# KolinGuo/MPlib

Hardware: AMD Instinct MI355X
Metric: configs/sec full collide() Panda-7DoF+10 boxes (higher is better)
Workload: dtype f64; 1 GPU; cfg3 panda_10boxes: 1048576 configs/GPU/step, 129 pairs, full self+world collide() with ACM filter; configs_per_gpu=1048576, pairs=129, mask_words=5, parallelism=dp1 (config shards, no data-path collective)

## Files before the change

include/mpgpu.h:

```cpp
#ifndef MPGPU_H
#define MPGPU_H

#include <stddef.h>
#include <stdint.h>

#ifdef __cplusplus
extern "C" {
#endif

#define MPG_VERSION_MAJOR 0
#define MPG_VERSION_MINOR 3

#define MPG_OK 0
#define MPG_E_INVALID 1
#define MPG_E_UNSUPPORTED 2
#define MPG_E_HIP 3
#define MPG_E_NOMEM 4
#define MPG_E_FAILED 5

#define MPG_MEM_HOST 0
#define MPG_MEM_DEVICE 1

#define MPG_JOINT_RX 0
#define MPG_JOINT_RY 1
// ... 206 lines not shown
#define MPG_SCREW_TRUNCATED 16
#define MPG_SCREW_SINGULAR 32
#define MPG_SCREW_ROT_PI 64

typedef struct mpg_screw_options {
  double qpos_step;
  int32_t max_waypoints;
} mpg_screw_options;

int mpg_screw_batch(mpg_world *world, int32_t link, const double *goal ,
                    const double *q_start , int64_t rows,
                    const mpg_screw_options *opt , double *path ,
                    int32_t *n_waypoints , uint8_t *status ,
                    int32_t *first_hit , int mem, void *stream);

int mpg_fcl_bvh_build(const double *vertices, int32_t n_vertices, const int32_t *triangles, int32_t n_triangles,
                      double *boxes, int32_t *links, int32_t *leaf_order);

int mpg_debug_sincos(const double *x, int64_t n, double *s, double *c, int device);

int mpg_latency_server_stats(mpg_world *world, int64_t *served, int64_t *starts, int64_t *fallbacks,
                             int32_t *state);

int mpg_synchronize(int device);

int mpg_device_count(int *count);
const char *mpg_last_error(void);
int mpg_last_error_copy(char *buf, size_t size);
const char *mpg_version(void);

#ifdef __cplusplus
}
#endif
#endif
```

mplib_amd/_capi.py:

```python
from __future__ import annotations

import ctypes
import os

_HERE = os.path.dirname(os.path.abspath(__file__))
LIB_PATH = os.path.join(_HERE, "lib", "libmpgpu.so")

MPG_OK, MPG_E_INVALID, MPG_E_UNSUPPORTED, MPG_E_HIP, MPG_E_NOMEM, MPG_E_FAILED = 0, 1, 2, 3, 4, 5
MPG_MEM_HOST, MPG_MEM_DEVICE = 0, 1
STAGES = ("cull", "bucket", "narrow")

(JOINT_RX, JOINT_RY, JOINT_RZ, JOINT_REVOLUTE_UNALIGNED, JOINT_PX, JOINT_PY, JOINT_PZ,
 JOINT_PRISMATIC_UNALIGNED, JOINT_RUBX, JOINT_RUBY, JOINT_RUBZ, JOINT_RUB_UNALIGNED) = range(12)
GEOM_CONVEX, GEOM_BOX, GEOM_SPHERE, GEOM_CAPSULE, GEOM_CYLINDER, GEOM_OCTREE, GEOM_MESH, GEOM_ELLIPSOID, GEOM_CONE = range(9)
GJK_LIBCCD, GJK_INDEP = 0, 1
LINK_FREE = -1

_I32P = ctypes.POINTER(ctypes.c_int32)
_F64P = ctypes.POINTER(ctypes.c_double)
_U8P = ctypes.POINTER(ctypes.c_uint8)
_U32P = ctypes.POINTER(ctypes.c_uint32)


class WorldDesc(ctypes.Structure):
# ... 117 lines not shown
                                                 ctypes.c_int64, ctypes.c_int, ctypes.c_void_p, ctypes.c_void_p,
                                                 ctypes.c_void_p, ctypes.c_void_p, ctypes.c_void_p, ctypes.c_int,
                                                 ctypes.c_void_p]),
    "mpg_fk_batch": (ctypes.c_int, [ctypes.c_void_p, ctypes.c_void_p, ctypes.c_int64, ctypes.c_void_p,
                                    ctypes.c_int, ctypes.c_void_p]),
    "mpg_ik_batch": (ctypes.c_int, [ctypes.c_void_p, ctypes.c_int32, ctypes.c_void_p, ctypes.c_int64, ctypes.c_int64,
                                    ctypes.c_void_p, ctypes.c_void_p, ctypes.POINTER(IkOptions), ctypes.c_void_p,
                                    ctypes.c_void_p, ctypes.c_void_p, ctypes.c_void_p, ctypes.c_int, ctypes.c_void_p]),
    "mpg_screw_batch": (ctypes.c_int, [ctypes.c_void_p, ctypes.c_int32, ctypes.c_void_p, ctypes.c_void_p, ctypes.c_int64,
                                       ctypes.POINTER(ScrewOptions), ctypes.c_void_p, ctypes.c_void_p, ctypes.c_void_p,
                                       ctypes.c_void_p, ctypes.c_int, ctypes.c_void_p]),
    "mpg_profile_enable": (ctypes.c_int, [ctypes.c_void_p, ctypes.c_int]),
    "mpg_profile_read": (ctypes.c_int, [ctypes.c_void_p, ctypes.POINTER(ctypes.c_double),
                                        ctypes.POINTER(ctypes.c_int64), ctypes.POINTER(ctypes.c_int64), ctypes.c_int]),
    "mpg_debug_collide_pairs": (ctypes.c_int, [ctypes.c_void_p, ctypes.c_int32, ctypes.c_int32, ctypes.c_int64,
                                                ctypes.c_void_p, ctypes.c_void_p, ctypes.c_void_p]),
    "mpg_debug_sincos": (ctypes.c_int, [ctypes.c_void_p, ctypes.c_int64, ctypes.c_void_p, ctypes.c_void_p,
                                        ctypes.c_int]),
    "mpg_fcl_bvh_build": (ctypes.c_int, [ctypes.c_void_p, ctypes.c_int32, ctypes.c_void_p, ctypes.c_int32,
                                         ctypes.c_void_p, ctypes.c_void_p, ctypes.c_void_p]),
    "mpg_latency_server_stats": (ctypes.c_int, [ctypes.c_void_p, ctypes.POINTER(ctypes.c_int64),
                                                ctypes.POINTER(ctypes.c_int64), ctypes.POINTER(ctypes.c_int64),
                                                ctypes.POINTER(ctypes.c_int32)]),
    "mpg_synchronize": (ctypes.c_int, [ctypes.c_int]),
    "mpg_device_count": (ctypes.c_int, [ctypes.POINTER(ctypes.c_int)]),
    "mpg_last_error": (ctypes.c_char_p, []),
    "mpg_last_error_copy": (ctypes.c_int, [ctypes.c_char_p, ctypes.c_size_t]),
    "mpg_version": (ctypes.c_char_p, []),
}

_lib = None


class MpgError(RuntimeError):
    pass


def lib() -> ctypes.CDLL:
    global _lib
    if _lib is None:
        if not os.path.exists(LIB_PATH):
            raise ImportError(f"mplib_amd: HIP library {LIB_PATH} is missing -- run `make -C mplib_amd` "
                              "(there is no CPU fallback)")
        try:
            import torch
        except ImportError:
# ... 19 lines not shown
```

mplib_amd/batch.py:

```python
from __future__ import annotations

import ctypes
from typing import Dict, Optional

import numpy as np

from . import _capi as C

_DESC_INT_FIELDS = ["joint_type", "joint_parent", "joint_q_source", "link_parent", "geom_type",
                    "geom_vertex_start", "geom_vertex_count", "moving_link", "moving_geom", "static_geom",
                    "pair_a", "pair_b"]
_DESC_F64_FIELDS = ["joint_axis", "joint_placement", "joint_q_const", "link_placement", "geom_param",
                    "vertices", "moving_offset", "static_transform"]


class DeviceWorld:

    def __init__(self, arrays: Dict[str, np.ndarray], device: int = 0, gjk_tolerance: float = 1e-6,
                 gjk_solver: int = C.GJK_LIBCCD):
        L = C.lib()
        self._keep = []

        def ip(name):
            a = np.ascontiguousarray(np.asarray(arrays[name], dtype=np.int32).reshape(-1))
# ... 67 lines not shown
        nf, far = ctypes.c_int32(0), ctypes.c_double(0.0)
        C.check(L.mpg_world_get_free_info(h, ctypes.byref(nf), ctypes.byref(far), None), "mpg_world_get_free_info")
        self.n_free = nf.value
        self.far_radius = far.value

    def close(self):
        if getattr(self, "_h", None):
            C.lib().mpg_world_destroy(self._h)
            self._h = None

    def __del__(self):
        try:
            self.close()
        except Exception:
            pass

    @property
    def handle(self):
        return self._h

    def set_small_batch_max(self, n: int):
        C.check(C.lib().mpg_set_small_batch_max(self._h, int(n)), "mpg_set_small_batch_max")

    def release_stream(self, stream: int):
        C.check(C.lib().mpg_release_stream(self._h, ctypes.c_void_p(int(stream))), "mpg_release_stream")

    def collide_batch(self, q, flags=None, pair_mask=None, stream: Optional[int] = None, free_pose=None):
        if hasattr(q, "data_ptr"):
            n = q.shape[0] if q.dim() > 1 else q.numel() // self.dof
            if flags is None:
                raise ValueError("device path needs preallocated flags (and optionally pair_mask)")
            mk = ctypes.c_void_p(pair_mask.data_ptr() if pair_mask is not None else 0)
            if free_pose is not None:
                rows = self._free_rows(free_pose.numel(), n)
                C.check(C.lib().mpg_collide_batch_free(self._h, ctypes.c_void_p(q.data_ptr()),
                                                       ctypes.c_void_p(free_pose.data_ptr()), rows, n,
                                                       ctypes.c_void_p(flags.data_ptr()), mk, C.MPG_MEM_DEVICE,
                                                       ctypes.c_void_p(stream or 0)), "mpg_collide_batch_free")
                return flags, pair_mask
            C.check(C.lib().mpg_collide_batch(self._h, ctypes.c_void_p(q.data_ptr()), n,
                                              ctypes.c_void_p(flags.data_ptr()), mk,
                                              C.MPG_MEM_DEVICE, ctypes.c_void_p(stream or 0)), "mpg_collide_batch")
            return flags, pair_mask
        qa = np.ascontiguousarray(np.asarray(q, dtype=np.float64)).reshape(-1, self.dof)
        n = qa.shape[0]
        fl = np.zeros(n, np.uint8)
# ... 183 lines not shown
```

mplib_amd/csrc/mpg_abi_world.h:

```cpp
#pragma once

const char* mpg_last_error(void) { return g_last_error.c_str(); }

int mpg_fcl_bvh_build(const double* vertices, int32_t n_vertices, const int32_t* triangles, int32_t n_triangles,
                      double* boxes, int32_t* links, int32_t* leaf_order) {
  if (n_triangles <= 0 || !vertices || !triangles || !boxes || !links || !leaf_order)
    return set_error(MPG_E_INVALID, "mpg_fcl_bvh_build: empty mesh or NULL buffer");
  for (int64_t i = 0; i < 3 * (int64_t)n_triangles; ++i)
    if (triangles[i] < 0 || triangles[i] >= n_vertices) return set_error(MPG_E_INVALID, "triangle vertex out of range");
  FclBvh B;
  B.box.resize(FB_STRIDE);
  B.link.resize(3);
  std::vector<int> prim((size_t)n_triangles);
  for (int t = 0; t < n_triangles; ++t) prim[t] = t;
  fcl_bvh_node(B, vertices, triangles, prim, 0, 0, n_triangles, 0);
  std::copy(B.box.begin(), B.box.end(), boxes);
  std::copy(B.link.begin(), B.link.end(), links);
  std::copy(prim.begin(), prim.end(), leaf_order);
  return (int)(B.link.size() / 3);
}

int mpg_last_error_copy(char* buf, size_t size) {
  const size_t len = g_last_error.size();
  if (buf && size > 0) {
// ... 46 lines not shown
  for (auto& mk : w->marks) {
    w->ev_pool.push_back(std::move(mk.a));
    w->ev_pool.push_back(std::move(mk.b));
  }
  w->marks.clear();
  for (int k = 0; k < MPG_NUM_STAGES; ++k) {
    if (k < n_stages) {
      if (ms) ms[k] = w->prof_ms[k];
      if (launches) launches[k] = w->prof_n[k];
      if (units) units[k] = u[k];
    }
    w->prof_ms[k] = 0.0;
    w->prof_n[k] = 0;
  }
  return MPG_OK;
}

int mpg_latency_server_stats(mpg_world* w, int64_t* served, int64_t* starts, int64_t* fallbacks, int32_t* state) {
  if (!w) return set_error(MPG_E_INVALID, "world is NULL");
  if (served) *served = w->srv_served;
  if (starts) *starts = w->srv_starts;
  if (fallbacks) *fallbacks = w->srv_fallbacks;
  if (state) *state = !(w->srv_mode && w->srv_ok) ? 0 : w->srv_broken ? 2 : 1;
  return MPG_OK;
}

int mpg_synchronize(int device) {
  HIP_TRY(hipSetDevice(device));
  HIP_TRY(hipDeviceSynchronize());
  return MPG_OK;
}

int mpg_world_create(const mpg_world_desc* d_in, int device, mpg_world** out) {
  if (!out) return set_error(MPG_E_INVALID, "out is NULL");
  *out = nullptr;
  int rc = validate(d_in);
  if (rc) return rc;
  mpg_world_desc dd = *d_in;
  std::vector<int32_t> lp_kin(dd.link_parent, dd.link_parent + dd.n_links);
  int n_free = 0;
  for (int32_t& p : lp_kin)
    if (p == MPG_LINK_FREE) {
      p = 0;
      ++n_free;
    }
  if (n_free) dd.link_parent = lp_kin.data();
// ... 312 lines not shown
  for (int m = 0; m < d->n_moving; ++m) off = std::max(off, std::sqrt(sq3(d->moving_offset + 12 * m + 9)));
  for (int g = 0; g < d->n_geoms; ++g) geo_r = std::max(geo_r, geom_rec[G_STRIDE * g + G_RADIUS] +
                                                                   std::sqrt(sq3(&geom_rec[G_STRIDE * g + G_OBB_C])));
  for (int s2 = 0; s2 < d->n_static; ++s2) stat_x = std::max(stat_x, std::sqrt(sq3(d->static_transform + 12 * s2 + 9)));
  double X = std::max(reach_x + off, stat_x) + geo_r;
  bp_margin = std::max(bp_margin, (float)(kFp32CullRel * X));
  double small_margin = may_mpr ? std::max(kSmallMargin, reach) : kSmallMargin;
  double far_r = 0.0;
  if (n_free) {
    const double link_r = std::sqrt(3.0) * reach_x + off + geo_r;
    const float quat_slack = (float)(4.0 * kFreeQuatTol * geo_r);
    bp_margin += quat_slack;
    small_margin += 4.0 * kFreeQuatTol * geo_r;
    for (int it = 0; it < 8; ++it) {
      far_r = (link_r + (double)bp_margin + 1e-6 * (1.0 + X)) * (1.0 + 1e-9);
      X = std::max(X, far_r + 2.0 * geo_r);
      bp_margin = std::max(bp_margin, (float)(kFp32CullRel * X) + quat_slack);
    }
    far_r = (link_r + (double)bp_margin + 1e-6 * (1.0 + X)) * (1.0 + 1e-9);
    X = std::max(X, far_r + 2.0 * geo_r);
  }
  const double pose_bound = reach_x;
  std::vector<std::array<double, 4>> ball(std::max(d->n_moving, 1));
  for (int m = 0; m < d->n_moving; ++m) {
    const int l = d->moving_link[m];
    const double* g = geom_rec.data() + G_STRIDE * d->moving_geom[m];
    const double* mo = d->moving_offset + 12 * m;
    const double* lp = d->link_placement + 12 * l;
    double a[3], bpt[3];
    for (int i = 0; i < 3; ++i)
      a[i] = mo[3 * i] * g[G_OBB_C] + mo[3 * i + 1] * g[G_OBB_C + 1] + mo[3 * i + 2] * g[G_OBB_C + 2] + mo[9 + i];
    for (int i = 0; i < 3; ++i) bpt[i] = lp[3 * i] * a[0] + lp[3 * i + 1] * a[1] + lp[3 * i + 2] * a[2] + lp[9 + i];
    const int cs = chain_start[l], cn = chain_len[l];
    double R = g[G_RADIUS];
    if (cn == 0) {
      ball[m] = {bpt[0], bpt[1], bpt[2], R};
      continue;
    }
    const int j1 = chain_joints[cs] - 1;
    const double* p1 = d->joint_placement + 12 * j1 + 9;
    R += travel[j1] + std::sqrt(sq3(bpt));
    for (int k = 1; k < cn; ++k) {
      const int j = chain_joints[cs + k] - 1;
      R += std::sqrt(sq3(d->joint_placement + 12 * j + 9)) + travel[j];
    }
    ball[m] = {p1[0], p1[1], p1[2], R * (1.0 + 1e-9) + 1e-9};
  }
  auto never_near = [&](int m, int sid) {
    const double* sr = static_rec.data() + (size_t)S_STRIDE * sid;
    const double* gs = geom_rec.data() + G_STRIDE * d->static_geom[sid];
    double e2 = 0.0;
    for (int k = 0; k < 3; ++k) {
      double t = 0.0;
      for (int i = 0; i < 3; ++i) t += (ball[m][i] - sr[S_OBBC + i]) * sr[S_R + 3 * i + k];
      const double ex = std::max(std::fabs(t) - gs[G_OBB_E + k], 0.0);
      e2 += ex * ex;
    }
    const double slack = 1e-6 * (1.0 + X);
    return std::sqrt(e2) - ball[m][3] > (double)bp_margin + slack;
  };
  std::vector<int> all_mask(std::max(W, 1), 0);
  for (int p = 0; p < d->n_pairs; ++p)
    if (!allowed[p]) all_mask[p >> 5] |= (int)(1u << (p & 31));
  const int ns = d->n_static;
  std::vector<int> sched_start(d->n_moving + 1, 0), sched_pair, sched_other, st_start(2 * (ns + 1), 0), st_m;
  std::vector<float> st_r;
  for (int m = 0; m < d->n_moving; ++m) {
    sched_start[m] = (int)sched_pair.size();
    for (int p = 0; p < d->n_pairs; ++p) {
// ... 4 lines not shown
      sched_pair.push_back(p);
      sched_other.push_back(hi);
      st_m.push_back(0);
      st_r.push_back(0.f);
    }
  }
  sched_start[d->n_moving] = (int)sched_pair.size();
  for (int g = 0; g < 2; ++g) {
    for (int sid = 0; sid < ns; ++sid) {
      st_start[g * (ns + 1) + sid] = (int)sched_pair.size();
      for (int m = 0; m < d->n_moving; ++m)
        for (int p = 0; p < d->n_pairs; ++p) {
          if (allowed[p]) continue;
          const int a = d->pair_a[p], b = d->pair_b[p];
          if (std::min(a, b) != m || std::max(a, b) != d->n_moving + sid) continue;
          if (never_near(m, sid) != (g == 1)) continue;
          sched_pair.push_back(p);
          sched_other.push_back(d->n_moving + sid);
          st_m.push_back(m);
          st_r.push_back(bpp.mobj[BM_STRIDE * m + BM_R]);
        }
    }
    st_start[g * (ns + 1) + ns] = (int)sched_pair.size();
  }
  if (sched_pair.empty()) {
    sched_pair.push_back(0);
    sched_other.push_back(0);
    st_m.push_back(0);
    st_r.push_back(0.f);
  }

  BlobBuilder bb;
  const size_t o_jt = bb.add(d->joint_type, d->n_joints);
  const size_t o_jp = bb.add(d->joint_parent, d->n_joints);
  const size_t o_jqs = bb.add(d->joint_q_source, d->n_joints);
  const size_t o_jqc = bb.add(d->joint_q_const, d->n_joints);
  const size_t o_ja = bb.add(d->joint_axis, 3 * (size_t)d->n_joints);
  const size_t o_jpl = bb.add(d->joint_placement, 12 * (size_t)d->n_joints);
  const size_t o_lp = bb.add(d->link_parent, d->n_links);
  const size_t o_lpl = bb.add(d->link_placement, 12 * (size_t)d->n_links);
  const size_t o_gt = bb.add(d->geom_type, d->n_geoms);
  const size_t o_gvs = bb.add(gstart.data(), gstart.size());
  const size_t o_gnv = bb.add(ngroups.data(), ngroups.size());
  std::vector<int> nvert(std::max(d->n_geoms, 1), 0);
  for (int g = 0; g < d->n_geoms; ++g) nvert[g] = d->geom_type[g] == MPG_GEOM_CONVEX ? d->geom_vertex_count[g] : 0;
  const size_t o_gnvt = bb.add(nvert.data(), nvert.size());
// ... 62 lines not shown
    r[SR_SH] = (bpp.pair_sh[2 * p] + 2) | ((bpp.pair_sh[2 * p + 1] + 2) << 16);
  }
  const size_t o_srr = bb.add(sched_rec.data(), sched_rec.size());
  const size_t o_olf = bb.add(oct_leaf.data(), oct_leaf.size());
  const size_t o_mtr = bb.add(mesh_tri.data(), mesh_tri.size());
  const size_t o_mnd = bb.add(mesh_node.data(), mesh_node.size());
  const size_t o_mln = bb.add(mesh_link.data(), mesh_link.size());
  const size_t o_mtt = bb.add(mesh_tree.data(), mesh_tree.size());
  const size_t o_lrec = bb.add(lat_rec.data(), lat_rec.size());
  const size_t o_fbb = bb.add(fbvh.box.data(), fbvh.box.size());
  const size_t o_fbl = bb.add(fbvh.link.data(), fbvh.link.size());
  const size_t o_fbr = bb.add(fb_root.data(), fb_root.size());
  const size_t o_tps = bb.add(tri_pos.data(), tri_pos.size());
  const size_t o_sob = bb.add(sobb.data(), sobb.size());
  const size_t o_ogr = bb.add(oct_grid.data(), oct_grid.size());
  const size_t o_oce = bb.add(oct_cells.data(), oct_cells.size());
  const size_t o_oli = bb.add(oct_list.data(), oct_list.size());
  const size_t o_opa = bb.add(oct_path.data(), oct_path.size());
  const size_t o_ode = bb.add(oct_depth.data(), oct_depth.size());
  std::vector<int> free_obj(n_free, 0);
  for (int m = 0; m < d->n_moving; ++m)
    if (d->moving_link[m] >= d->n_links - n_free) free_obj[d->moving_link[m] - (d->n_links - n_free)] = m;
  const size_t o_fob = n_free ? bb.add(free_obj.data(), free_obj.size()) : 0;

  std::unique_ptr<mpg_world> w(new mpg_world());
  w->device = device;
  w->n_geoms = d->n_geoms;
  w->geom_type_h.assign(d->geom_type, d->geom_type + d->n_geoms);
  w->block = block;
  w->lds_bytes = lds;
  w->blob_bytes = bb.bytes.size();
  {
    uint64_t h = 1469598103934665603ull;
    for (const char c : bb.bytes) h = (h ^ (uint8_t)c) * 1099511628211ull;
    w->snapshot_hash = h;
  }
  HIP_TRY(w->blob.reserve(w->blob_bytes));
  HIP_TRY(hipMemcpy(w->blob.get(), bb.bytes.data(), w->blob_bytes, hipMemcpyHostToDevice));
  char* base = w->blob.get();
  DevWorld& dw = w->dw;
  dw.nj = d->n_joints;
  dw.dof = d->dof;
  dw.n_links = d->n_links;
  dw.n_geoms = d->n_geoms;
  dw.n_moving = d->n_moving;
  dw.n_static = d->n_static;
// ... 96 lines not shown
    w->has_closed_form |= pair_cf[p] != CF_NONE && !allowed[p];
    w->has_octree |= pair_cf[p] == CF_OCTREE && !allowed[p];
    w->octree_first |= pair_cf[p] == CF_OCTREE && !allowed[p] && obj_geom_type(d, d->pair_a[p]) == MPG_GEOM_OCTREE;
    w->any_closed_form |= pair_cf[p] != CF_NONE && cf_class(pair_cf[p]) == CLS_CLOSED;
    w->any_octree |= pair_cf[p] == CF_OCTREE;
    w->has_mesh |= pair_cf[p] == CF_MESH && !allowed[p];
    w->any_mesh |= pair_cf[p] == CF_MESH;
    w->any_gjk |= pair_cf[p] == CF_GJK;
    w->has_octree2 |= !allowed[p] && obj_geom_type(d, d->pair_a[p]) == MPG_GEOM_OCTREE &&
                      obj_geom_type(d, d->pair_b[p]) == MPG_GEOM_OCTREE;
  }
  dw.static_T = to_cptr<double>(base + o_sT);
  dw.link_chain_start = to_cptr<int>(base + o_cs);
  dw.link_chain_len = to_cptr<int>(base + o_cl);
  dw.chain_joints = to_cptr<int>(base + o_cj);
  auto I = [&](size_t o) { return to_cptr<int>(base + o); };
  dw.sched_start = I(o_ss);
  dw.sched_pair = I(o_sp);
  dw.sched_other = I(o_so);
  dw.sched_rec = I(o_srr);
  dw.st_start = I(o_sts);
  dw.st_m = I(o_stm);
  dw.st_r = to_cptr<float>(base + o_str);
  auto F = [&](size_t o) { return to_cptr<float>(base + o); };
  BpView& bp = dw.bp;
  bp.nj = d->n_joints;
  bp.n_links = d->n_links;
  bp.n_moving = d->n_moving;
  bp.n_static = d->n_static;
  bp.n_saves = bpp.n_saves;
  bp.joint_type = dw.joint_type;
  bp.joint_q_source = dw.joint_q_source;
  bp.joint_q_const = dw.joint_q_const;
  bp.jsrc = I(o_bjs);
  bp.jsave = I(o_bjv);
  bp.jaxis = F(o_bja);
  bp.jplace = F(o_bjp);
  bp.link_start = I(o_bls);
  bp.link_order = I(o_blo);
  bp.lplace = F(o_blp);
  bp.obj_start = I(o_bos);
  bp.obj_order = I(o_boo);
  bp.moving_link = dw.moving_link;
  bp.moff = F(o_bmo);
  bp.mobj = F(o_bmb);
  bp.sobj = F(o_bsb);
// ... 158 lines not shown
```

mplib_amd/csrc/mpg_broadphase.h:

```cpp
#pragma once
#include <cmath>
#include <vector>

#include "mpg_math.h"
#include "../../include/mpgpu.h"

namespace mpg {

constexpr float kBpMargin = 1e-4f;
constexpr double kFp32CullRel = 4e-6;
constexpr float kFarPark = 1e15f;
constexpr double kFreeQuatTol = 1e-6;
constexpr double kDefaultTravel = 10.0;

#ifdef __clang__
#define MPG_FP32_CONTRACT _Pragma("clang fp contract(fast)")
#else
#define MPG_FP32_CONTRACT
#endif

enum { BM_C = 0, BM_E = 3, BM_R = 6, BM_STRIDE = 8 };
enum { BS_C = 0, BS_R = 3, BS_E = 12, BS_STRIDE = 16 };

struct BpView {
// ... 642 lines not shown
  b.jsrc = to_cptr<int>(P.jsrc.data());
  b.jsave = to_cptr<int>(P.jsave.data());
  b.jaxis = to_cptr<float>(P.jaxis.data());
  b.jplace = to_cptr<float>(P.jplace.data());
  b.link_start = to_cptr<int>(P.link_start.data());
  b.link_order = to_cptr<int>(P.link_order.data());
  b.lplace = to_cptr<float>(P.lplace.data());
  b.obj_start = to_cptr<int>(P.obj_start.data());
  b.obj_order = to_cptr<int>(P.obj_order.data());
  b.moving_link = to_cptr<int>(d->moving_link);
  b.moff = to_cptr<float>(P.moff.data());
  b.mobj = to_cptr<float>(P.mobj.data());
  b.sobj = to_cptr<float>(P.sobj.data());
  b.jkind = to_cptr<int>(P.jkind.data());
  b.jobj_start = to_cptr<int>(P.jobj_start.data());
  b.jobj_order = to_cptr<int>(P.jobj_order.data());
  b.oplace = to_cptr<float>(P.oplace.data());
  b.oquat = to_cptr<float>(P.oquat.data());
  b.ocen = to_cptr<float>(P.ocen.data());
  b.shtab = to_cptr<float>(P.shtab.data());
  return b;
}

}
```

mplib_amd/csrc/mpg_fk.h:

```cpp
#pragma once
#include "mpg_math.h"
#include "mpg_broadphase.h"
#include "mpg_hullcells.h"
#include "../../include/mpgpu.h"

namespace mpg {

constexpr int kMaxJoints = 32;

enum { G_PARAM = 0, G_INTERIOR = 4, G_OBB_C = 7, G_OBB_E = 10, G_RADIUS = 13, G_VMAX = 14, G_AABB_E = 15, G_STRIDE = 18 };
enum { S_ROT = 0, S_ROTINV = 4, S_POS = 8, S_OBBC = 11, S_R = 14, S_STRIDE = 23 };

struct DevWorld {
  int nj, dof, n_links, n_geoms, n_moving, n_static, n_pairs, W;
  double mpr_tol;
  float bp_margin;
  float sh_margin;
  double small_margin;
  int debug_mode;
  unsigned long long* stats;
  MPG_INLINE bool dbg(int k) const {
#ifdef MPG_DIAG
    return debug_mode == k;
#else
// ... 30 lines not shown
  cptr<int> wcell_pre;
  int walk_subk;
  cptr<int> moving_link;
  cptr<int> moving_geom;
  cptr<double> moving_offset;
  cptr<int> static_geom;
  cptr<double> static_rec;
  cptr<int> pair_a;
  cptr<int> pair_b;
  cptr<int> pair_allowed;
  cptr<int> pair_cf;
  cptr<double> static_T;
  cptr<int> link_chain_start;
  cptr<int> link_chain_len;
  cptr<int> chain_joints;
  BpView bp;
  cptr<int> sched_start;
  cptr<int> sched_pair;
  cptr<int> sched_other;
  cptr<int> sched_rec;
  cptr<int> st_start;
  cptr<int> st_m;
  cptr<float> st_r;
  int n_prism;
  cptr<double> prism_bound;
  double pose_bound;
  cptr<int> all_mask;
  unsigned long long* big_vis;
  int* big_busy;
  int big_slots, big_words;
  cptr<double> oct_leaf;
  cptr<double> oct_grid;
  cptr<int> oct_cells;
  cptr<int> oct_list;
  cptr<uint64_t> oct_path;
  cptr<int> oct_depth;
  cptr<double> mesh_tri;
  cptr<double> mesh_node;
  cptr<int> mesh_link;
  cptr<int> mesh_tree;
  cptr<double> fb_box;
  cptr<int> fb_link;
  cptr<int> fb_root;
  cptr<int> tri_pos;
  cptr<double> sobb;
  cptr<double> lat_rec;
// ... 120 lines not shown
```

mplib_amd/csrc/mpg_kernels.hip:

```cpp

#include <hip/hip_runtime.h>

#include <algorithm>
#include <atomic>
#include <chrono>
#include <cfloat>
#include <cstdio>
#include <cstdlib>
#include <cstring>
#include <limits>
#include <map>
#include <memory>
#include <mutex>
#include <string>
#include <thread>
#include <vector>

#include "../../include/mpgpu.h"
#include "mpg_math.h"
#include "mpg_fk.h"
#include "mpg_ik.h"
#include "mpg_screw.h"
#include "mpg_bucket.h"
#include "mpg_hostpipe.h"
// ... 911 lines not shown
  const unsigned long long bal = __ballot(keep);
  const uint32_t ns = (uint32_t)__popcll(bal);
  if (ns) {
    const uint32_t rank = __builtin_amdgcn_mbcnt_hi((uint32_t)(bal >> 32), __builtin_amdgcn_mbcnt_lo((uint32_t)bal, 0u));
    const uint32_t dst = keep ? npend + rank : npend + ns + (lane - rank);
    const uint32_t recv = (uint32_t)__builtin_amdgcn_ds_permute((int)((dst & 63u) << 2), (int)e);
    if (npend + ns >= 64u) {
      support_drain<BLOCK>(w, cen, rq, cap, cfg0, survw, lane >= npend ? recv : pend, 64, wbase, lane);
      pend = recv;
      npend = npend + ns - 64u;
    } else {
      if (lane >= npend && lane < npend + ns) pend = recv;
      npend += ns;
    }
  }
  __builtin_amdgcn_wave_barrier();
}

template <int BLOCK, bool FROM_POSES>
__global__ __launch_bounds__(BLOCK) __attribute__((amdgpu_waves_per_eu(4, 4))) void cull_kernel(DevWorld w, const double* __restrict__ in, long long n,
                                                    uint8_t* __restrict__ flags, uint32_t* __restrict__ masks,
                                                    uint32_t* __restrict__ surv, float* __restrict__ rq,
                                                    double* __restrict__ sc, long long cap,
                                                    uint32_t* __restrict__ cnt, int n_tiles) {
  extern __shared__ __attribute__((aligned(16))) float lds_f[];
  float* cen = lds_f;
  float* save = cen + (size_t)w.n_moving * 3 * BLOCK;
  uint32_t* survw = reinterpret_cast<uint32_t*>(save + (size_t)max(w.bp.n_saves - kRegSaves, 0) * 12 * BLOCK);
  const int tid = threadIdx.x;
  uint32_t* queue = survw + (size_t)w.W * BLOCK + (tid >> 6) * kQueue;
  const uint32_t lane = lane_id();
  const int wbase = tid & ~63;
  const long long cfg0 = (long long)blockIdx.x * BLOCK;
  const long long cfg = cfg0 + tid;
  const bool live = cfg < n;
  const long long c = live ? cfg : n - 1;
  if (live) {
    flags[cfg] = 0;
    if (masks)
      for (int k = 0; k < w.W; ++k) masks[cfg * w.W + k] = 0u;
  }
  for (int k = 0; k < w.W; ++k) survw[k * BLOCK + tid] = 0u;
  if (w.dbg(14)) return;

  auto store_obj = [&](int m, const float* q, const float* c) {
    if (live && !w.dbg(13)) {
      float* r = rq + (size_t)m * 4 * cap + cfg;
// ... 106 lines not shown
    }
    uint32_t any_kb = kb;
#pragma unroll
    for (int sh = 1; sh < 64; sh <<= 1) any_kb |= (uint32_t)__shfl_xor((int)any_kb, sh);
    any_kb = __builtin_amdgcn_readfirstlane(any_kb);
    while (any_kb) {
      const int i = __builtin_ctz(any_kb);
      any_kb &= any_kb - 1u;
      const bool keep = (kb >> i) & 1u;
      const unsigned long long bal = __ballot(keep);
      if (keep) {
        const uint32_t rank =
            __builtin_amdgcn_mbcnt_hi((uint32_t)(bal >> 32), __builtin_amdgcn_mbcnt_lo((uint32_t)bal, 0u));
        queue[(tail + rank) & (kQueue - 1)] = ((uint32_t)(eb + i) << 6) | lane;
      }
      tail += (uint32_t)__popcll(bal);
      if (tail - head >= 64) {
        sat_drain<BLOCK>(w, cen, rq, cap, cfg0, survw, queue, head, 64, wbase, lane, pend, npend);
        head += 64;
      }
    }
  };
  const int ns = w.n_static;
  for (int g = 0; g < (FROM_POSES ? 2 : 1) && !w.dbg(12); ++g) {
    const int E0 = w.st_start[g * (ns + 1)], E1 = w.st_start[g * (ns + 1) + ns];
    if (E0 == E1) continue;
    int eb = E0;
    uint32_t kb = 0u;
    for (int sid = 0; sid < ns; ++sid) {
      const int e0 = w.st_start[g * (ns + 1) + sid], e1 = w.st_start[g * (ns + 1) + sid + 1];
      if (e0 == e1) continue;
      const cptr<float> rec = w.bp.sobj + BS_STRIDE * sid;
      float sr[BS_STRIDE];
#pragma unroll
      for (int k = 0; k < BS_STRIDE; ++k) sr[k] = rec[k];
#pragma unroll 2
      for (int e = e0; e < e1; ++e) {
        if (e - eb == 32) {
          push(eb, kb);
          eb = e;
          kb = 0u;
        }
        const float* rm = cen + (size_t)w.st_m[e] * 3 * BLOCK + tid;
        const float cm[3] = {rm[0], rm[BLOCK], rm[2 * BLOCK]};
        kb |= (uint32_t)!fsphere_obb_separated(cm, w.st_r[e], sr, w.bp_margin) << (e - eb);
      }
    }
    push(eb, kb);
  }
  for (int m = 0; m < w.n_moving; ++m) {
    const int e0 = w.sched_start[m], e1 = w.sched_start[m + 1];
    if (e0 == e1) continue;
    const float* rm = cen + (size_t)m * 3 * BLOCK + tid;
// ... 5159 lines not shown
```

mplib_amd/csrc/mpg_streams_host.h:

```cpp
#pragma once

void release_stream_locked(mpg_world* w, hipStream_t s) {
  const auto wi = w->ws.find(s);
  const auto si = w->sides.find(s);
  const auto ki = w->ik_ws.find(s);
  const auto ci = w->screw_ws.find(s);
  if (wi == w->ws.end() && si == w->sides.end() && ki == w->ik_ws.end() && ci == w->screw_ws.end()) return;
  hipDeviceSynchronize();
  if (ki != w->ik_ws.end()) w->ik_ws.erase(ki);
  if (ci != w->screw_ws.end()) w->screw_ws.erase(ci);
  if (wi != w->ws.end()) w->ws.erase(wi);
  if (si != w->sides.end()) {
    w->ws.erase(si->second.side.get());
    w->sides.erase(si);
  }
}

void evict_streams_locked(mpg_world* w) {
  std::map<hipStream_t, uint64_t> callers;
  for (auto& kv : w->ws) callers[kv.first] = kv.second.last;
  for (auto& kv : w->sides) {
    callers.erase(kv.second.side.get());
    uint64_t& t = callers[kv.first];
    t = std::max(t, kv.second.last);
// ... 73 lines not shown
  int stage;
  Event a;
  StageTimer(mpg_world* w_, hipStream_t s_, int st) : w(w_), s(s_), stage(st) {
    if (!w->prof) return;
    std::lock_guard<std::mutex> lk(w->prof_mu);
    a = prof_event(w);
    if (a) hipEventRecord(a.get(), s);
  }
  void stop() {
    if (!a) return;
    std::lock_guard<std::mutex> lk(w->prof_mu);
    Event b = prof_event(w);
    if (!b) return;
    hipEventRecord(b.get(), s);
    w->marks.push_back({stage, std::move(a), std::move(b)});
  }
  ~StageTimer() { stop(); }
};

struct ContactOut {
  double *depth, *normal, *pos;
};

template <bool FROM_POSES>
int launch_collide(mpg_world* w, const double* in, long long n, uint8_t* flags, uint32_t* masks, hipStream_t stream,
                   const ContactOut* co = nullptr) {
  if (n == 0) return MPG_OK;
  StreamPin pin(w, stream);
  const long long chunk = std::min<long long>(n, w->max_chunk);
  mpg_world::Workspace* owner = nullptr;
  int rc = get_workspace(w, stream, chunk, &owner);
  if (rc) return rc;
  uint32_t *const surv = owner->surv.get(), *const cnt = owner->cnt.get(), *const part = owner->part.get(),
                  *const grp = owner->grp.get(), *const seg_len = owner->seg_len.get(),
                  *const seg_start = owner->seg_start.get(), *const prefix = owner->prefix.get(),
                  *const cand = owner->cand.get();
  float* const rq = owner->rq.get();
  double* const sc = owner->sc.get();
  const long long cap = owner->cap;
  const size_t row = FROM_POSES ? (size_t)w->dw.n_links * 7 : (size_t)w->dw.dof;
  for (long long off = 0; off < n; off += chunk) {
    const long long m = std::min(chunk, n - off);
    const double* qin = in + off * row;
    uint8_t* fl = flags + off;
    uint32_t* mk = masks ? masks + off * w->dw.W : nullptr;
    const unsigned grid = (unsigned)((m + w->block - 1) / w->block);
    const int n_tiles = (int)((m + 63) / 64);
    StageTimer t_cull(w, stream, MPG_STAGE_CULL);
    if (w->prof) w->prof_cfg += m;
#ifndef MPG_DIAG
    if (w->dw.W * 8 > kQueue)
#endif
      HIP_TRY(hipMemsetAsync(cnt, 0, sizeof(uint32_t) * bk_cnt_words(w->dw.W, m), stream));
    switch (w->block) {
      case 256:
        hipLaunchKernelGGL((cull_kernel<256, FROM_POSES>), dim3(grid), dim3(256), w->lds_bytes, stream, w->dw, qin,
                           m, fl, mk, surv, rq, sc, cap, cnt, n_tiles);
        break;
      case 128:
        hipLaunchKernelGGL((cull_kernel<128, FROM_POSES>), dim3(grid), dim3(128), w->lds_bytes, stream, w->dw, qin,
                           m, fl, mk, surv, rq, sc, cap, cnt, n_tiles);
        break;
      default:
        hipLaunchKernelGGL((cull_kernel<64, FROM_POSES>), dim3(grid), dim3(64), w->lds_bytes, stream, w->dw, qin, m,
                           fl, mk, surv, rq, sc, cap, cnt, n_tiles);
        break;
    }
    HIP_TRY(hipGetLastError());
    t_cull.stop();
    StageTimer t_bucket(w, stream, MPG_STAGE_BUCKET);
    const int n_ranges = bk_ranges(n_tiles), n_groups = bk_groups(n_ranges);
    const long long tw = (long long)n_tiles * w->dw.W;
    const unsigned gb = (unsigned)((tw + 3) / 4);
    const bool fold = bk_fold_sum(n_ranges, w->dw.W);
    if (!fold) {
      hipLaunchKernelGGL(range_sum_kernel, dim3(n_groups), dim3(256), 0, stream, cnt, n_tiles, w->dw.W, part, grp);
      HIP_TRY(hipGetLastError());
    }
    hipLaunchKernelGGL(range_scan_kernel, dim3(1), dim3(1024), 0, stream, fold ? cnt : nullptr, n_tiles, w->dw.W,
                       part, grp, n_groups, w->dw.n_pairs, seg_len, seg_start, prefix,
                       w->prof ? w->prof_units.get() : nullptr, (uint32_t)(4 * w->narrow_blocks));
    HIP_TRY(hipGetLastError());
    hipLaunchKernelGGL(scatter_kernel, dim3(gb), dim3(256), 0, stream, surv, m, cap, w->dw.n_pairs, w->dw.W,
                       n_tiles, cnt, part, grp, seg_start, cand);
    HIP_TRY(hipGetLastError());
    t_bucket.stop();
    StageTimer t_narrow(w, stream, MPG_STAGE_NARROW);
    const long long want_waves = (m * std::max(w->dw.n_pairs, 1) + kTaskMin - 1) / kTaskMin;
// ... 101 lines not shown
```

mplib_amd/csrc/mpg_world.h:

```cpp
#pragma once

struct mpg_world {
  ~mpg_world();
  int device = 0;
  DevWorld dw{};
  int n_geoms = 0;
  std::vector<int> geom_type_h;
  DevBuf<char> blob;
  size_t blob_bytes = 0;
  uint64_t snapshot_hash = 0;
  Stream own_stream;
  Event gather_ev;
  DevBuf<unsigned long long> big_vis;
  DevBuf<int> big_busy;
  DevBuf<unsigned long long> stats;
  DevBuf<double> free_dev;
  int block = 128;
  size_t lds_bytes = 0;
  std::mutex host_mu;
  DevBuf<double> d_q, d_out;
  DevBuf<uint8_t> d_flags;
  DevBuf<uint32_t> d_masks;
  size_t cap_cfg = 0;
  size_t cap_out = 0;
  struct Workspace {
    DevBuf<uint32_t> surv;
    DevBuf<uint32_t> cnt;
    DevBuf<uint32_t> part;
    DevBuf<uint32_t> grp;
    DevBuf<uint32_t> seg_len;
    DevBuf<uint32_t> seg_start;
    DevBuf<uint32_t> prefix;
    DevBuf<uint32_t> cand;
    DevBuf<float> rq;
    DevBuf<double> sc;
    DevBuf<double> links;
    long long links_cap = 0;
    long long cap = 0;
    uint64_t last = 0;
// ... 153 lines not shown
```

Baseline: 1.664 billion configs/s.

## Add per-object spatial lookup grids to precompute moving-vs-world broadphase pair masks

Adds a precomputed 3D voxel grid for each moving object that has a moderate number of static partners. On first use the host fills each cell with a bitmask of the static obstacles that could be within reach of that object's centre, then uploads it. The cull kernel now looks up the cell from the object centre and pushes those bitmask words straight into the survivor stream, in place of running per-pair OBB/sphere tests against every static box. This trades the per-config arithmetic for one table lookup but adds a lazy, mutex-guarded host build at first call, extra device memory, and a more conservative cull because the cell is coarse, which may send more pairs to the narrow phase.

```diff
diff --git a/include/mpgpu.h b/include/mpgpu.h
--- a/include/mpgpu.h
+++ b/include/mpgpu.h
@@ -252,6 +252,9 @@
 int mpg_latency_server_stats(mpg_world *world, int64_t *served, int64_t *starts, int64_t *fallbacks,
                              int32_t *state);
 
+int mpg_cull_grid_info(const mpg_world *world, int32_t *objects, int64_t *cells, int32_t *built, double *cell_edge,
+                       int32_t cap, int32_t *object, int32_t *partners, double *box);
+
 int mpg_synchronize(int device);
 
 int mpg_device_count(int *count);
diff --git a/mplib_amd/_capi.py b/mplib_amd/_capi.py
--- a/mplib_amd/_capi.py
+++ b/mplib_amd/_capi.py
@@ -163,6 +163,9 @@
     "mpg_latency_server_stats": (ctypes.c_int, [ctypes.c_void_p, ctypes.POINTER(ctypes.c_int64),
                                                 ctypes.POINTER(ctypes.c_int64), ctypes.POINTER(ctypes.c_int64),
                                                 ctypes.POINTER(ctypes.c_int32)]),
+    "mpg_cull_grid_info": (ctypes.c_int, [ctypes.c_void_p, ctypes.POINTER(ctypes.c_int32), ctypes.POINTER(ctypes.c_int64),
+                                          ctypes.POINTER(ctypes.c_int32), ctypes.POINTER(ctypes.c_double), ctypes.c_int32,
+                                          ctypes.c_void_p, ctypes.c_void_p, ctypes.c_void_p]),
     "mpg_synchronize": (ctypes.c_int, [ctypes.c_int]),
     "mpg_device_count": (ctypes.c_int, [ctypes.POINTER(ctypes.c_int)]),
     "mpg_last_error": (ctypes.c_char_p, []),
diff --git a/mplib_amd/batch.py b/mplib_amd/batch.py
--- a/mplib_amd/batch.py
+++ b/mplib_amd/batch.py
@@ -113,6 +113,20 @@
     def set_small_batch_max(self, n: int):
         C.check(C.lib().mpg_set_small_batch_max(self._h, int(n)), "mpg_set_small_batch_max")
 
+    def cull_grid_info(self) -> dict:
+        n, cells, built = ctypes.c_int32(0), ctypes.c_int64(0), ctypes.c_int32(0)
+        edge = ctypes.c_double(0.0)
+        L = C.lib()
+        C.check(L.mpg_cull_grid_info(self._h, ctypes.byref(n), ctypes.byref(cells), ctypes.byref(built),
+                                     ctypes.byref(edge), 0, None, None, None), "mpg_cull_grid_info")
+        obj = np.zeros(n.value, np.int32)
+        part = np.zeros(n.value, np.int32)
+        box = np.zeros((n.value, 6))
+        C.check(L.mpg_cull_grid_info(self._h, None, None, None, None, n.value, obj.ctypes.data_as(ctypes.c_void_p),
+                                     part.ctypes.data_as(ctypes.c_void_p), box.ctypes.data_as(ctypes.c_void_p)),
+                "mpg_cull_grid_info")
+        return dict(objects=obj, partners=part, box=box, cells=cells.value, cell_edge=edge.value, built=bool(built.value))
+
     def release_stream(self, stream: int):
         C.check(C.lib().mpg_release_stream(self._h, ctypes.c_void_p(int(stream))), "mpg_release_stream")
 
diff --git a/mplib_amd/csrc/mpg_abi_world.h b/mplib_amd/csrc/mpg_abi_world.h
--- a/mplib_amd/csrc/mpg_abi_world.h
+++ b/mplib_amd/csrc/mpg_abi_world.h
@@ -92,6 +92,22 @@
   if (starts) *starts = w->srv_starts;
   if (fallbacks) *fallbacks = w->srv_fallbacks;
   if (state) *state = !(w->srv_mode && w->srv_ok) ? 0 : w->srv_broken ? 2 : 1;
+  return MPG_OK;
+}
+
+int mpg_cull_grid_info(const mpg_world* w, int32_t* objects, int64_t* cells, int32_t* built, double* cell_edge,
+                       int32_t cap, int32_t* object, int32_t* partners, double* box) {
+  if (!w) return set_error(MPG_E_INVALID, "world is NULL");
+  const mpg_world::GridInfo& g = w->grid_info;
+  if (objects) *objects = (int32_t)g.object.size();
+  if (cells) *cells = g.cells;
+  if (built) *built = w->grid_ready.load(std::memory_order_acquire) ? 1 : 0;
+  if (cell_edge) *cell_edge = g.h;
+  for (int32_t i = 0; i < cap && i < (int32_t)g.object.size(); ++i) {
+    if (object) object[i] = g.object[i];
+    if (partners) partners[i] = g.partners[i];
+    if (box) std::copy(g.box.begin() + 6 * i, g.box.begin() + 6 * i + 6, box + 6 * i);
+  }
   return MPG_OK;
 }
 
@@ -450,6 +466,7 @@
   }
   const double pose_bound = reach_x;
   std::vector<std::array<double, 4>> ball(std::max(d->n_moving, 1));
+  std::vector<double> ball_rc(std::max(d->n_moving, 1), 0.0);
   for (int m = 0; m < d->n_moving; ++m) {
     const int l = d->moving_link[m];
     const double* g = geom_rec.data() + G_STRIDE * d->moving_geom[m];
@@ -473,6 +490,7 @@
       R += std::sqrt(sq3(d->joint_placement + 12 * j + 9)) + travel[j];
     }
     ball[m] = {p1[0], p1[1], p1[2], R * (1.0 + 1e-9) + 1e-9};
+    ball_rc[m] = (R - g[G_RADIUS]) * (1.0 + 1e-9) + 1e-9;
   }
   auto never_near = [&](int m, int sid) {
     const double* sr = static_rec.data() + (size_t)S_STRIDE * sid;
@@ -523,6 +541,69 @@
         }
     }
     st_start[g * (ns + 1) + ns] = (int)sched_pair.size();
+  }
+  BpGridPlan gplan;
+  std::vector<int> gst_start, grid_i;
+  std::vector<float> grid_f;
+  {
+    const double slack = kFp32CullRel * X + 1e-6;
+    for (int m = 0; m < d->n_moving && n_free == 0; ++m) {
+      BpGridObj o;
+      o.m = m;
+      o.r = (double)bpp.mobj[BM_STRIDE * m + BM_R];
+      for (int k = 0; k < 3; ++k) {
+        o.lo[k] = ball[m][k] - (ball_rc[m] + slack);
+        o.hi[k] = ball[m][k] + (ball_rc[m] + slack);
+      }
+      for (int sid = 0; sid < ns; ++sid)
+        for (int p = 0; p < d->n_pairs; ++p) {
+          if (allowed[p]) continue;
+          const int a = d->pair_a[p], b = d->pair_b[p];
+          if (std::min(a, b) != m || std::max(a, b) != d->n_moving + sid || never_near(m, sid)) continue;
+          o.sid.push_back(sid);
+          o.pair.push_back(p);
+        }
+      if (bp_grid_candidate(o.sid.size())) gplan.obj.push_back(std::move(o));
+    }
+    bp_grid_choose(gplan, X, (double)bp_margin);
+  }
+  if (!gplan.obj.empty()) {
+    std::vector<char> gridded(d->n_moving, 0);
+    std::vector<int> E;
+    for (const BpGridObj& o : gplan.obj) {
+      gridded[o.m] = 1;
+      E.push_back((int)sched_pair.size());
+      for (size_t k = 0; k < o.sid.size(); ++k) {
+        sched_pair.push_back(o.pair[k]);
+        sched_other.push_back(d->n_moving + o.sid[k]);
+        st_m.push_back(o.m);
+        st_r.push_back(bpp.mobj[BM_STRIDE * o.m + BM_R]);
+      }
+    }
+    E.push_back((int)sched_pair.size());
+    bp_grid_records(gplan, E, grid_f, grid_i);
+    gst_start.assign(ns + 1, 0);
+    for (int sid = 0; sid < ns; ++sid) {
+      gst_start[sid] = (int)sched_pair.size();
+      for (int m = 0; m < d->n_moving; ++m)
+        for (int p = 0; p < d->n_pairs && !gridded[m]; ++p) {
+          if (allowed[p]) continue;
+          const int a = d->pair_a[p], b = d->pair_b[p];
+          if (std::min(a, b) != m || std::max(a, b) != d->n_moving + sid || never_near(m, sid)) continue;
+          sched_pair.push_back(p);
+          sched_other.push_back(d->n_moving + sid);
+          st_m.push_back(m);
+          st_r.push_back(bpp.mobj[BM_STRIDE * m + BM_R]);
+        }
+    }
+    gst_start[ns] = (int)sched_pair.size();
+    gplan.sobb.assign((size_t)15 * ns, 0.0);
+    for (int sid = 0; sid < ns; ++sid) {
+      const float* r = bpp.sobj.data() + BS_STRIDE * sid;
+      double* S = gplan.sobb.data() + 15 * (size_t)sid;
+      for (int k = 0; k < 3; ++k) S[k] = r[BS_C + k], S[12 + k] = r[BS_E + k];
+      for (int k = 0; k < 9; ++k) S[3 + k] = r[BS_R + k];
+    }
   }
   if (sched_pair.empty()) {
     sched_pair.push_back(0);
@@ -631,6 +712,10 @@
   for (int m = 0; m < d->n_moving; ++m)
     if (d->moving_link[m] >= d->n_links - n_free) free_obj[d->moving_link[m] - (d->n_links - n_free)] = m;
   const size_t o_fob = n_free ? bb.add(free_obj.data(), free_obj.size()) : 0;
+  const bool has_grid = !gplan.obj.empty();
+  const size_t o_ggf = has_grid ? bb.add(grid_f.data(), grid_f.size()) : 0;
+  const size_t o_ggi = has_grid ? bb.add(grid_i.data(), grid_i.size()) : 0;
+  const size_t o_gst = has_grid ? bb.add(gst_start.data(), gst_start.size()) : 0;
 
   std::unique_ptr<mpg_world> w(new mpg_world());
   w->device = device;
@@ -773,6 +858,19 @@
   dw.st_start = I(o_sts);
   dw.st_m = I(o_stm);
   dw.st_r = to_cptr<float>(base + o_str);
+  dw.n_grid = has_grid ? (int)(grid_i.size() / GI_STRIDE) : 0;
+  dw.grid_f = to_cptr<float>(base + o_ggf);
+  dw.grid_i = I(o_ggi);
+  dw.gst_start = I(o_gst);
+  for (const BpGridObj& o : gplan.obj) {
+    w->grid_info.object.push_back(o.m);
+    w->grid_info.partners.push_back((int)o.sid.size());
+    for (int k = 0; k < 3; ++k) w->grid_info.box.push_back((double)o.o[k]);
+    for (int k = 0; k < 3; ++k) w->grid_info.box.push_back((double)o.o[k] + o.n[k] * gplan.h);
+  }
+  w->grid_info.cells = has_grid ? gplan.cells : 0;
+  w->grid_info.h = has_grid ? gplan.h : 0.0;
+  w->grid_plan = std::move(gplan);
   auto F = [&](size_t o) { return to_cptr<float>(base + o); };
   BpView& bp = dw.bp;
   bp.nj = d->n_joints;
diff --git a/mplib_amd/csrc/mpg_broadphase.h b/mplib_amd/csrc/mpg_broadphase.h
--- a/mplib_amd/csrc/mpg_broadphase.h
+++ b/mplib_amd/csrc/mpg_broadphase.h
@@ -688,4 +688,150 @@
   return b;
 }
 
-}
+constexpr int kGridMaxPartners = 32;
+constexpr int kGridMinPartners = 6;
+constexpr long long kGridBudget = 1ll << 19;
+constexpr double kGridMinH = 0.02;
+constexpr double kGridMaxH = 0.08;
+constexpr int kGridBlock = 8;
+constexpr int kGridGroup = 4;
+enum { GF_O = 0, GF_INVH = 3, GF_N = 4, GF_STRIDE = 8 };
+enum { GI_M = 0, GI_NX = 1, GI_NY = 2, GI_CELL0 = 3, GI_E = 4, GI_NP = 5, GI_FULL = 6, GI_STRIDE = 8 };
+
+template <class PF, class PI>
+MPG_INLINE int bp_grid_cell(PF gf, PI gi, const float* c) {
+  const float inv = gf[GF_INVH];
+  const float fx = (c[0] - gf[GF_O]) * inv, fy = (c[1] - gf[GF_O + 1]) * inv, fz = (c[2] - gf[GF_O + 2]) * inv;
+  const bool in = fx >= 0.f && fx < gf[GF_N] && fy >= 0.f && fy < gf[GF_N + 1] && fz >= 0.f && fz < gf[GF_N + 2];
+  const int ix = in ? (int)fx : 0, iy = in ? (int)fy : 0, iz = in ? (int)fz : 0;
+  return in ? gi[GI_CELL0] + (iz * gi[GI_NY] + iy) * gi[GI_NX] + ix : -1;
+}
+
+struct BpGridObj {
+  int m = 0;
+  double lo[3] = {0, 0, 0}, hi[3] = {0, 0, 0};
+  double r = 0.0;
+  std::vector<int> sid, pair;
+  int n[3] = {1, 1, 1};
+  float o[3] = {0.f, 0.f, 0.f};
+  long long cell0 = 0;
+};
+struct BpGridPlan {
+  std::vector<BpGridObj> obj;
+  std::vector<double> sobb;
+  double h = 0.0;
+  float inv_h = 0.f;
+  double thr_pad = 0.0;
+  double cell_pad = 0.0;
+  long long cells = 0;
+};
+
+inline bool bp_grid_candidate(size_t partners) { return partners >= (size_t)kGridMinPartners && partners <= (size_t)kGridMaxPartners; }
+
+inline long long bp_grid_layout(BpGridPlan& G, double h, long long budget) {
+  G.inv_h = (float)(1.0 / h);
+  G.h = 1.0 / (double)G.inv_h;
+  G.cells = 0;
+  for (BpGridObj& o : G.obj) {
+    o.cell0 = G.cells;
+    long long c = 1;
+    for (int k = 0; k < 3; ++k) {
+      o.o[k] = (float)o.lo[k];
+      o.n[k] = (int)std::min(1048576.0, std::max(1.0, std::ceil((o.hi[k] - (double)o.o[k]) / G.h)));
+      c = std::min(c * o.n[k], budget + 1);
+    }
+    G.cells += c;
+  }
+  return G.cells;
+}
+
+inline void bp_grid_choose(BpGridPlan& G, double coord_bound, double margin, long long budget = kGridBudget) {
+  auto vol = [](const BpGridObj& o) { return (o.hi[0] - o.lo[0]) * (o.hi[1] - o.lo[1]) * (o.hi[2] - o.lo[2]); };
+  for (bool fits = false; !fits && !G.obj.empty();) {
+    for (double h = kGridMinH; h <= kGridMaxH && !fits; h *= 1.0625) fits = bp_grid_layout(G, h, budget) <= budget;
+    if (fits) break;
+    size_t big = 0;
+    for (size_t i = 1; i < G.obj.size(); ++i)
+      if (vol(G.obj[i]) > vol(G.obj[big])) big = i;
+    G.obj.erase(G.obj.begin() + big);
+  }
+  if (G.obj.empty()) bp_grid_layout(G, kGridMinH, budget);
+  int nmax = 1;
+  for (const BpGridObj& o : G.obj) nmax = std::max(nmax, std::max(o.n[0], std::max(o.n[1], o.n[2])));
+  G.thr_pad = margin + kFp32CullRel * coord_bound + 1e-9;
+  G.cell_pad = G.h * nmax * 3e-7 + kFp32CullRel * coord_bound;
+}
+
+inline double bp_grid_gap(const double* q, const double* a, const double* S) {
+  double g2 = 0.0, d2 = 0.0;
+  for (int k = 0; k < 3; ++k) {
+    double t = 0.0, w = 0.0;
+    for (int i = 0; i < 3; ++i) {
+      t += (q[i] - S[i]) * S[3 + 3 * i + k];
+      w += a[i] * std::fabs(S[3 + 3 * i + k]);
+    }
+    const double g = std::max(std::fabs(t) - w - S[12 + k], 0.0), ex = std::max(std::fabs(t) - S[12 + k], 0.0);
+    g2 += g * g;
+    d2 += ex * ex;
+  }
+  return std::max(std::sqrt(g2), std::sqrt(d2) - std::sqrt(a[0] * a[0] + a[1] * a[1] + a[2] * a[2]) * (1.0 + 1e-6));
+}
+
+inline void bp_grid_fill(const BpGridPlan& G, std::vector<uint32_t>& words) {
+  words.assign((size_t)std::max(G.cells, 1ll), 0u);
+  for (const BpGridObj& o : G.obj) {
+    const int np = (int)o.sid.size();
+    const double thr = o.r + G.thr_pad;
+    int near[kGridMaxPartners];
+    for (int bz = 0; bz < o.n[2]; bz += kGridBlock)
+      for (int by = 0; by < o.n[1]; by += kGridBlock)
+        for (int bx = 0; bx < o.n[0]; bx += kGridBlock) {
+          const int b0[3] = {bx, by, bz};
+          int b1[3];
+          double q[3], a[3];
+          for (int k = 0; k < 3; ++k) {
+            b1[k] = std::min(b0[k] + kGridBlock, o.n[k]);
+            q[k] = (double)o.o[k] + 0.5 * (b0[k] + b1[k]) * G.h;
+            a[k] = 0.5 * (b1[k] - b0[k]) * G.h + G.cell_pad;
+          }
+          int nn = 0;
+          for (int k = 0; k < np; ++k)
+            if (!(bp_grid_gap(q, a, G.sobb.data() + 15 * (size_t)o.sid[k]) > thr)) near[nn++] = k;
+          if (nn == 0) continue;
+          const double ac[3] = {0.5 * G.h + G.cell_pad, 0.5 * G.h + G.cell_pad, 0.5 * G.h + G.cell_pad};
+          for (int iz = b0[2]; iz < b1[2]; ++iz)
+            for (int iy = b0[1]; iy < b1[1]; ++iy)
+              for (int ix = b0[0]; ix < b1[0]; ++ix) {
+                const double qc[3] = {(double)o.o[0] + (ix + 0.5) * G.h, (double)o.o[1] + (iy + 0.5) * G.h,
+                                      (double)o.o[2] + (iz + 0.5) * G.h};
+                uint32_t wd = 0u;
+                for (int j = 0; j < nn; ++j)
+                  if (!(bp_grid_gap(qc, ac, G.sobb.data() + 15 * (size_t)o.sid[near[j]]) > thr)) wd |= 1u << near[j];
+                words[(size_t)(o.cell0 + ((long long)iz * o.n[1] + iy) * o.n[0] + ix)] = wd;
+              }
+        }
+  }
+}
+
+inline void bp_grid_records(const BpGridPlan& G, const std::vector<int>& E, std::vector<float>& gf, std::vector<int>& gi) {
+  const size_t n = (G.obj.size() + kGridGroup - 1) / kGridGroup * kGridGroup;
+  gf.assign(n * GF_STRIDE, 0.f);
+  gi.assign(n * GI_STRIDE, 0);
+  for (size_t i = 0; i < G.obj.size(); ++i) {
+    const BpGridObj& o = G.obj[i];
+    float* f = gf.data() + GF_STRIDE * i;
+    int* r = gi.data() + GI_STRIDE * i;
+    for (int k = 0; k < 3; ++k) f[GF_O + k] = o.o[k], f[GF_N + k] = (float)o.n[k];
+    f[GF_INVH] = G.inv_h;
+    r[GI_M] = o.m;
+    r[GI_NX] = o.n[0];
+    r[GI_NY] = o.n[1];
+    r[GI_CELL0] = (int)o.cell0;
+    r[GI_E] = E[i];
+    r[GI_NP] = (int)o.sid.size();
+    r[GI_FULL] = (int)(o.sid.size() >= 32 ? ~0u : (1u << o.sid.size()) - 1u);
+  }
+  for (size_t i = G.obj.size(); i < n; ++i) gi[GI_STRIDE * i + GI_E] = E.empty() ? 0 : E.back();
+}
+
+}
diff --git a/mplib_amd/csrc/mpg_fk.h b/mplib_amd/csrc/mpg_fk.h
--- a/mplib_amd/csrc/mpg_fk.h
+++ b/mplib_amd/csrc/mpg_fk.h
@@ -76,6 +76,10 @@
   cptr<int> st_start;
   cptr<int> st_m;
   cptr<float> st_r;
+  int n_grid;
+  cptr<float> grid_f;
+  cptr<int> grid_i;
+  cptr<int> gst_start;
   int n_prism;
   cptr<double> prism_bound;
   double pose_bound;
diff --git a/mplib_amd/csrc/mpg_kernels.hip b/mplib_amd/csrc/mpg_kernels.hip
--- a/mplib_amd/csrc/mpg_kernels.hip
+++ b/mplib_amd/csrc/mpg_kernels.hip
@@ -957,7 +957,8 @@
                                                     uint8_t* __restrict__ flags, uint32_t* __restrict__ masks,
                                                     uint32_t* __restrict__ surv, float* __restrict__ rq,
                                                     double* __restrict__ sc, long long cap,
-                                                    uint32_t* __restrict__ cnt, int n_tiles) {
+                                                    uint32_t* __restrict__ cnt, int n_tiles,
+                                                    const uint32_t* __restrict__ grid) {
   extern __shared__ __attribute__((aligned(16))) float lds_f[];
   float* cen = lds_f;
   float* save = cen + (size_t)w.n_moving * 3 * BLOCK;
@@ -1110,13 +1111,46 @@
     }
   };
   const int ns = w.n_static;
+  const bool use_grid = !FROM_POSES && grid != nullptr && w.n_grid > 0 && !w.dbg(12) && !w.dbg(15);
+  if (use_grid) {
+    int eb = w.grid_i[GI_E], fill = 0;
+    unsigned long long acc = 0ull;
+    for (int g0 = 0; g0 < w.n_grid; g0 += kGridGroup) {
+      uint32_t wd[kGridGroup];
+#pragma unroll
+      for (int j = 0; j < kGridGroup; ++j) {
+        const cptr<float> gf = w.grid_f + GF_STRIDE * (g0 + j);
+        const cptr<int> gi = w.grid_i + GI_STRIDE * (g0 + j);
+        const float* rm = cen + (size_t)gi[GI_M] * 3 * BLOCK + tid;
+        const float cm[3] = {rm[0], rm[BLOCK], rm[2 * BLOCK]};
+        const int cell = bp_grid_cell(gf, gi, cm);
+        const uint32_t x = grid[cell < 0 ? 0 : cell];
+        wd[j] = cell < 0 ? (uint32_t)gi[GI_FULL] : x;
+      }
+      static_assert(kGridGroup == 4, "the selection below names four words");
+#pragma unroll 1
+      for (int j = 0; j < kGridGroup; ++j) {
+        const uint32_t x = j == 0 ? wd[0] : j == 1 ? wd[1] : j == 2 ? wd[2] : wd[3];
+        acc |= (unsigned long long)x << fill;
+        fill += w.grid_i[GI_STRIDE * (g0 + j) + GI_NP];
+        const bool last = g0 + j + 1 == w.n_grid;
+        while (fill >= 32 || (last && fill > 0)) {
+          push(eb, (uint32_t)acc);
+          acc >>= 32;
+          eb += 32;
+          fill = max(fill - 32, 0);
+        }
+      }
+    }
+  }
   for (int g = 0; g < (FROM_POSES ? 2 : 1) && !w.dbg(12); ++g) {
-    const int E0 = w.st_start[g * (ns + 1)], E1 = w.st_start[g * (ns + 1) + ns];
+    const cptr<int> sts = use_grid ? w.gst_start : w.st_start + g * (ns + 1);
+    const int E0 = sts[0], E1 = sts[ns];
     if (E0 == E1) continue;
     int eb = E0;
     uint32_t kb = 0u;
     for (int sid = 0; sid < ns; ++sid) {
-      const int e0 = w.st_start[g * (ns + 1) + sid], e1 = w.st_start[g * (ns + 1) + sid + 1];
+      const int e0 = sts[sid], e1 = sts[sid + 1];
       if (e0 == e1) continue;
       const cptr<float> rec = w.bp.sobj + BS_STRIDE * sid;
       float sr[BS_STRIDE];
diff --git a/mplib_amd/csrc/mpg_streams_host.h b/mplib_amd/csrc/mpg_streams_host.h
--- a/mplib_amd/csrc/mpg_streams_host.h
+++ b/mplib_amd/csrc/mpg_streams_host.h
@@ -119,11 +119,38 @@
   double *depth, *normal, *pos;
 };
 
+inline int grid_words_for(mpg_world* w, const uint32_t** out) {
+  *out = nullptr;
+  if (w->dw.n_grid == 0) return MPG_OK;
+  if (!w->grid_ready.load(std::memory_order_acquire)) {
+    std::lock_guard<std::mutex> lk(w->grid_mu);
+    if (!w->grid_ready.load(std::memory_order_relaxed)) {
+      const auto t0 = std::chrono::steady_clock::now();
+      std::vector<uint32_t> words;
+      bp_grid_fill(w->grid_plan, words);
+      HIP_TRY(w->grid_words.reserve(words.size()));
+      HIP_TRY(hipMemcpy(w->grid_words.get(), words.data(), sizeof(uint32_t) * words.size(), hipMemcpyHostToDevice));
+      w->grid_plan = BpGridPlan();
+      w->grid_build_ms = std::chrono::duration<double, std::milli>(std::chrono::steady_clock::now() - t0).count();
+      if (std::getenv("MPG_STATS"))
+        std::fprintf(stderr, "[mpg] lookup grids: %zu cells built in %.1f ms\n", words.size(), w->grid_build_ms);
+      w->grid_ready.store(true, std::memory_order_release);
+    }
+  }
+  *out = w->grid_words.get();
+  return MPG_OK;
+}
+
 template <bool FROM_POSES>
 int launch_collide(mpg_world* w, const double* in, long long n, uint8_t* flags, uint32_t* masks, hipStream_t stream,
                    const ContactOut* co = nullptr) {
   if (n == 0) return MPG_OK;
   StreamPin pin(w, stream);
+  const uint32_t* gwords = nullptr;
+  if (!FROM_POSES) {
+    const int grc = grid_words_for(w, &gwords);
+    if (grc) return grc;
+  }
   const long long chunk = std::min<long long>(n, w->max_chunk);
   mpg_world::Workspace* owner = nullptr;
   int rc = get_workspace(w, stream, chunk, &owner);
@@ -152,15 +179,15 @@
     switch (w->block) {
       case 256:
         hipLaunchKernelGGL((cull_kernel<256, FROM_POSES>), dim3(grid), dim3(256), w->lds_bytes, stream, w->dw, qin,
-                           m, fl, mk, surv, rq, sc, cap, cnt, n_tiles);
+                           m, fl, mk, surv, rq, sc, cap, cnt, n_tiles, gwords);
         break;
       case 128:
         hipLaunchKernelGGL((cull_kernel<128, FROM_POSES>), dim3(grid), dim3(128), w->lds_bytes, stream, w->dw, qin,
-                           m, fl, mk, surv, rq, sc, cap, cnt, n_tiles);
+                           m, fl, mk, surv, rq, sc, cap, cnt, n_tiles, gwords);
         break;
       default:
         hipLaunchKernelGGL((cull_kernel<64, FROM_POSES>), dim3(grid), dim3(64), w->lds_bytes, stream, w->dw, qin, m,
-                           fl, mk, surv, rq, sc, cap, cnt, n_tiles);
+                           fl, mk, surv, rq, sc, cap, cnt, n_tiles, gwords);
         break;
     }
     HIP_TRY(hipGetLastError());
diff --git a/mplib_amd/csrc/mpg_world.h b/mplib_amd/csrc/mpg_world.h
--- a/mplib_amd/csrc/mpg_world.h
+++ b/mplib_amd/csrc/mpg_world.h
@@ -15,6 +15,17 @@
   DevBuf<int> big_busy;
   DevBuf<unsigned long long> stats;
   DevBuf<double> free_dev;
+  BpGridPlan grid_plan;
+  DevBuf<uint32_t> grid_words;
+  std::mutex grid_mu;
+  std::atomic<bool> grid_ready{false};
+  double grid_build_ms = 0.0;
+  struct GridInfo {
+    std::vector<int> object, partners;
+    std::vector<double> box;
+    long long cells = 0;
+    double h = 0.0;
+  } grid_info;
   int block = 128;
   size_t lds_bytes = 0;
   std::mutex host_mu;
```

Result: faster. 1.730 billion configs/s, median of 6 (+4.0%).
